# bevanda/Learning-Based-MPC

Measured on AMD Instinct MI355X. Metric: QP-steps/s (whole node) at N=20 Moore-Greitzer; KKT-residual vs MATLAB ref, higher is better.
Workload: dtype f64; 1 GPU; C2: MG LMPC (F1) N=20, 616-row terminal set, batch 1024 per GPU, fp64; batch_per_gpu=1024, horizon=20, parallelism=dp1, streams=1

## Files before the change

### learning-based-mpc_amd/csrc/bqp_api.cpp

```cpp
#include <hip/hip_runtime.h>
#include <math.h>
#include <stdio.h>
#include <stdlib.h>
#include <string.h>

#include <algorithm>
#include <vector>

#include "../../include/bqp.h"
#include "bqp_internal.h"
#include "bqp_layout.h"

namespace layout = bqp::layout;

struct DevBuf {
    void* p = nullptr;
    size_t bytes = 0;
    hipError_t reserve(size_t n) {
        if (n <= bytes) return hipSuccess;
        if (p) hipFree(p);
        p = nullptr;
        bytes = 0;
        hipError_t e = hipMalloc(&p, n);
        if (e == hipSuccess) bytes = n;
// ... 268 lines not shown
    auto shared_layout = [&](bool single) {
        Shared o;
        o.lng = !single && N + 1 > 64;
        o.hpsh = mp > 0 && D->shp == 0;
        o.bndsh = o.lng && D->sxb == 0 && D->sub == 0;
        const int nbr = (N + 1) * 2 * (nx + nu);
        int sh = (o.lng || hinst) ? 0 : (N + 1) * hstride;
        o.sh_F = sh;
        sh += fpi ? 0 : nv * mpad;
        o.sh_hp = o.hpsh ? sh : -1;
        sh += o.hpsh ? mpad : 0;
        o.sh_bnd = o.bndsh ? sh : -1;
        sh += o.bndsh ? nbr : 0;
        o.doubles = (sh + 1) & ~1;
        return o;
    };
    const Shared L64 = shared_layout(f32), L32 = shared_layout(true);
    const bool lng = L64.lng;
    auto fit_wpb = [&](bool single, int& wpb) -> bool {
        const Shared& S = single ? L32 : L64;
        const int shared_doubles = S.doubles;
        const int per_wave = single ? bqp::ocp_wave_lds_doubles_f32(N, nx, nu, np, mpad, fpi, false, S.hpsh, false, hinst)
                                    : bqp::ocp_wave_lds_doubles(N, nx, nu, np, mpad, fpi, S.lng, S.hpsh, S.bndsh, hinst);
        const size_t lds_budget = (160 * 1024 - 256) / (single ? sizeof(float) : sizeof(double));
        wpb = (N + 1 > 64) ? 2 : 4;
        if (const char* e = getenv("BQP_OCP_WPB")) {
            const int v = atoi(e);
            if (v >= 1 && v <= 8) wpb = v;
        }
        while (wpb > 1 && (size_t)shared_doubles + (size_t)wpb * per_wave > lds_budget) --wpb;
        return (size_t)shared_doubles + (size_t)per_wave <= lds_budget;
    };
    int wpb = 1, wpb32 = 1;
    if (!fit_wpb(f32, wpb)) return BQP_E_UNSUPPORTED;
    if (mixed && !fit_wpb(true, wpb32)) return BQP_E_UNSUPPORTED;
    const layout::Work WL = work_layout(N, nv, mpad, batch);
    HIP_TRY(h->work.reserve(WL.bytes));
    double* Hd = layout::at<double>(h->work.p, WL.H);
    double* Fd = layout::at<double>(h->work.p, WL.F);
    double* Sd = layout::at<double>(h->work.p, WL.stats);
    int* polneed = layout::at<int>(h->work.p, WL.marks);
    int* queues = layout::at<int>(h->work.p, WL.queues);
    const double* Hinst = nullptr;
    if (hinst) {
        HIP_TRY(h->wwork.reserve(sizeof(double) * (size_t)batch * (N + 1) * hstride));
        HIP_TRY(bqp::launch_ocp_prep_h(D->W, D->sW, batch, nx, nu, np, N, hstride, (double*)h->wwork.p, st));
        Hinst = (const double*)h->wwork.p;
    }
    void* Pg = nullptr;
    if (lng) {
        HIP_TRY(h->pwork.reserve(sizeof(double) * (size_t)batch * (N + 1) * bqp::ocp_pstride(nx + np)));
        Pg = h->pwork.p;
    }
    HIP_TRY(bqp::launch_ocp_prep(D->W, mp > 0 ? D->Fp : D->W, nx, nu, np, N, mp, d->poly_stage,
                                 hstride, mpad, Hd, Fd, queues, st));
    bqp::OcpKernelArgs a;
    memset(&a, 0, sizeof(a));
    a.queue = queues;
    a.N = N; a.mp = mp; a.kp = d->poly_stage; a.batch = batch; a.wpb = wpb;
    const Shared& LS = f32 ? L32 : L64;
    a.hstride = hstride; a.mpad = mpad; a.shared_doubles = LS.doubles;
    a.Pg = Pg; a.sh_F = LS.sh_F; a.sh_hp = LS.sh_hp; a.sh_bnd = LS.sh_bnd; a.H_inst = Hinst;
    a.max_iter = o.max_iter; a.tol_stat = o.tol_stat; a.tol_feas = o.tol_feas;
    a.tol_comp = o.tol_comp; a.tau = o.tau;
    a.polish = o.polish < 0 ? 0 : (o.polish == 0 ? 1 : std::min(o.polish, 2));
    a.pol_need = polneed;
    a.H = Hd; a.Fp = Fd;
    a.A = D->A; a.B = D->B; a.c = D->c; a.w = D->w; a.xlb = D->xlb; a.xub = D->xub;
    a.ulb = D->ulb; a.uub = D->uub; a.hp = mp > 0 ? D->hp : Hd; a.x0 = D->x0;
    a.sA = D->sA; a.sB = D->sB; a.sc = D->sc; a.sw = D->sw; a.sxb = D->sxb; a.sub = D->sub;
    a.shp = D->shp; a.sx0 = D->sx0;
    if (fpi) { a.Fp_inst = D->Fp; a.sFp = D->sFp; }
    a.x = x; a.u = u; a.theta = theta; a.fval = fval; a.exitflag = exitflag; a.stats = Sd;
    if (duals) {
        a.pi_out = duals->pi; a.lamx_out = duals->lam_x; a.lamu_out = duals->lam_u;
        a.lamp_out = duals->lam_p;
    }
#ifdef BQP_STAMPS
    a.stamps = layout::at<double>(h->work.p, WL.stamps);
    h->last_batch = batch;
#endif
    HIP_TRY(hipEventRecord(h->ev0, st));
    if (mixed) {
        const int hf = bqp::ocp_hand_floats(N, nx, nu, np, mp);
        if (hf <= 0) return BQP_E_UNSUPPORTED;
        const layout::Hwork HL(hf, batch);
        const size_t hrec = HL.stride;
        HIP_TRY(h->hwork.reserve(HL.bytes));
        float* hb = layout::at<float>(h->hwork.p, HL.records);
        int* hflag = layout::at<int>(h->hwork.p, HL.flags);
        int* hit = layout::at<int>(h->hwork.p, HL.iters);
        int* c2flag = layout::at<int>(h->hwork.p, HL.cont);
        h->mixed_flags = hflag;
        h->mixed_cont = c2flag;
        h->mixed_batch = batch;
        bqp::OcpKernelArgs a1 = a;
        a1.wpb = wpb32;
        a1.shared_doubles = L32.doubles; a1.sh_F = L32.sh_F; a1.sh_hp = L32.sh_hp; a1.sh_bnd = L32.sh_bnd;
        a1.max_iter = o32.max_iter; a1.tol_stat = o32.tol_stat; a1.tol_feas = o32.tol_feas;
        a1.tol_comp = o32.tol_comp;
        a1.exitflag = hflag;
        a1.hand_out = hb; a1.hand_it = hit; a1.hand_stride = (int64_t)hrec;
        a1.pi_out = a1.lamx_out = a1.lamu_out = a1.lamp_out = nullptr;
        a1.queue = queues + 1;
        HIP_TRY(bqp::launch_ocp_f32(a1, nx, nu, np, st));
        a.hand_in = hb; a.hand_flag = hflag; a.hand_it = hit; a.hand_stride = (int64_t)hrec;
        HIP_TRY(bqp::launch_ocp(a, nx, nu, np, st));
        HIP_TRY(hipMemcpyAsync(c2flag, exitflag, sizeof(int) * batch, hipMemcpyDeviceToDevice, st));
        bqp::OcpKernelArgs a3 = a;
        a3.hand_in = nullptr; a3.hand_it = nullptr; a3.redo_flag = hflag;
        a3.queue = nullptr;
        HIP_TRY(bqp::launch_ocp(a3, nx, nu, np, st));
    } else if (f32) {
        HIP_TRY(bqp::launch_ocp_f32(a, nx, nu, np, st));
    } else {
        HIP_TRY(bqp::launch_ocp(a, nx, nu, np, st));
    }
    if (!f32 && a.polish > 0) HIP_TRY(bqp::launch_ocp(a, nx, nu, np, st, true));
    HIP_TRY(hipEventRecord(h->ev1, st));
    h->timed = true;
// ... 675 lines not shown
```

### learning-based-mpc_amd/csrc/bqp_internal.h

```cpp
#pragma once
#include <hip/hip_runtime.h>
#include <stdint.h>

namespace bqp {

constexpr int STATS_W = 7;

constexpr int OCP_QUEUES = 4;
struct OcpKernelArgs {
    int N, mp, kp, batch, wpb, hstride, mpad, shared_doubles, max_iter;
    int* queue;
    double tol_stat, tol_feas, tol_comp, tau;
    const double* H;
    const double* Fp;
    const double *A, *B, *c, *w, *xlb, *xub, *ulb, *uub, *hp, *x0;
    int64_t sA, sB, sc, sw, sxb, sub, shp, sx0;
    double *x, *u, *theta, *fval;
    int* exitflag;
    double* stats;
    double *pi_out, *lamx_out, *lamu_out, *lamp_out;
    double* stamps;
    float* hand_out;
    const float* hand_in;
    const int* hand_flag;
    int* hand_it;
    int64_t hand_stride;
    const int* redo_flag;
    const double* Fp_inst;
    int64_t sFp;
    void* Pg;
    int sh_F, sh_hp, sh_bnd;
    const double* H_inst;
    int polish;
    int* pol_need;
};

bool ocp_supported(int nx, int nu, int np);
int ocp_rpl_for(int mp);
int ocp_bpl_for(int N, int nx, int nu);
int ocp_hand_floats(int N, int nx, int nu, int np, int mp);
int ocp_wave_lds_doubles(int N, int nx, int nu, int np, int mpad, bool fpi, bool lng, bool hpsh,
                         bool bndsh, bool hinst);
int ocp_pstride(int ns);
hipError_t launch_ocp(const OcpKernelArgs& a, int nx, int nu, int np, hipStream_t st, bool pol = false);
int ocp_wave_lds_doubles_f32(int N, int nx, int nu, int np, int mpad, bool fpi, bool lng,
                             bool hpsh, bool bndsh, bool hinst);
hipError_t launch_ocp_f32(const OcpKernelArgs& a, int nx, int nu, int np, hipStream_t st, bool pol = false);
hipError_t launch_ocp_prep(const double* W, const double* Fp, int nx, int nu, int np, int N,
                           int mp, int kp, int hstride, int mpad, double* Hout, double* Fout,
                           int* qzero, hipStream_t st);
hipError_t launch_ocp_prep_h(const double* W, int64_t sW, int batch, int nx, int nu, int np,
                             int N, int hstride, double* Hout, hipStream_t st);
hipError_t launch_ocp_finalize(const double* stats, int batch, void* out, hipStream_t st);

struct DenseKernelArgs {
    int n, m, me, batch, max_iter, mrows;
    double tol_stat, tol_feas, tol_comp, tau;
    const double *H, *f, *A, *b, *Aeq, *beq, *lb, *ub;
    int64_t sH, sf, sA, sb, sAeq, sbeq, slb, sub;
    double *x, *fval, *lam_ineqlin, *lam_eqlin, *lam_lower, *lam_upper;
    int* exitflag;
    double* stats;
    double* work;
    int64_t work_stride;
    int polish;
    const int* pol_it;
    int pol_stall;
    const int* skip;
    int res_every;
};

int dense_work_doubles(int n, int m, int me);
hipError_t launch_dense(const DenseKernelArgs& a, hipStream_t st);
hipError_t launch_dense_symmetrize(double* H, int n, int count, int64_t stride, hipStream_t st);

struct LbmpcArgs {
    int N, n, nr, m, q, n_run, term_learned, batch, ntrial, max_iter, wrows;
    double hinv2, lam_nw, tol_step, tol_stat;
    const double *A, *B, *K, *Lq, *Lr, *Lp, *Lt, *LAM, *PSI, *xs;
    const double* data; int64_t sdata;
    const double* x0; int64_t sx0;
    const double* Ain;
    const double* bin; int64_t sbin;
    double* z;
    double* d;
    double* lam;
    double *Jr, *er;
    double *H, *f, *bsh;
    double *cost0, *costT, *stat, *cprev;
    int *qpflag, *flag, *done, *iters, *ndone;
    int hess;
    double *Jr2, *Tr2;
    int* hused;
};

hipError_t launch_nw_oracle(int batch, int q, const double* data, int64_t sdata, const double* xi,
                            double* g, double* dg, double bw, double lam, hipStream_t st);
bool lbmpc_hess_fits(int n);
bool lbmpc_supported(int nx, int nu, int np, int n, int q);
hipError_t launch_lbmpc_rollout(const LbmpcArgs& a, int gn, hipStream_t st);
hipError_t launch_lbmpc_normal(const LbmpcArgs& a, hipStream_t st);
hipError_t launch_lbmpc_update(const LbmpcArgs& a, hipStream_t st);
hipError_t launch_lbmpc_hess(const LbmpcArgs& a, hipStream_t st);
// ... 29 lines not shown
```

### learning-based-mpc_amd/csrc/bqp_ocp.hip

```cpp
#include <hip/hip_runtime.h>
#include <math.h>
#include <stdint.h>
#include <stdlib.h>

#include "bqp_internal.h"
#include "bqp_lanes.h"
#include "bqp_wave.h"

namespace bqp {

#ifdef BQP_F32
typedef float real;
typedef float2 real2;
#define BQP_SFX _f32
namespace sp {
#else
typedef double real;
typedef double2 real2;
#define BQP_SFX
namespace dp {
#endif
#define BQP_CAT2(a, b) a##b
#define BQP_CAT(a, b) BQP_CAT2(a, b)

// ... 557 lines not shown
        for (int t = 0; t < VPL; ++t) {
            o.h[t] = BQP_HV(vr[t] * NV + vc[t]);
            o.d[t] = W[L.Dx + k * NV + vr[t]];
        }
    };
    auto ht = [&](int k, const HRaw& o, int t) __attribute__((always_inline)) -> real {
        real v = o.h[t] + (vr[t] == vc[t] ? o.d[t] : real(0));
        if (k == kp) v += W[L.FD + vr[t] * NV + vc[t]];
        return v;
    };
    real pu[PST];
    auto read_p = [&](int k) __attribute__((always_inline)) {
        wave_sync();
        const real2* src = reinterpret_cast<const real2*>(W + L.P + (LNG ? (k & 1) : k) * PST);
#pragma unroll
        for (int q = 0; q < PST / 2; ++q) {
            const real2 t2 = src[q];
            pu[2 * q] = t2.x;
            pu[2 * q + 1] = t2.y;
        }
    };
    auto Pm = [&](int a_, int b_) __attribute__((always_inline)) -> real { return pu[pk_idx(NS, a_, b_)]; };
    auto factor = [&]() __attribute__((always_inline)) -> bool {
        HRaw raw, nxt;
        {
            load_h(N, raw);
            const real v0 = ht(N, raw, 0);
            if (fquad && fql == 0) {
                W[L.P + (LNG ? (N & 1) : N) * PST + fq] = v0;
                if constexpr (LNG) Pgl[N * PST + fq] = v0;
            }
        }
        read_p(N);
        bool ok = true;
        auto fstage = [&](int k, const HRaw& raw) __attribute__((always_inline)) {
            real mv[VPL];
#pragma unroll
            for (int t = 0; t < VPL; ++t) {
                real sp0 = 0, sp1 = 0, sp2 = 0, sp3 = 0;
#pragma unroll
                for (int m = 0; m < NPK; ++m) {
                    if ((m & 3) == 0) sp0 = fmar(cf[t][m], pu[m], sp0);
                    if ((m & 3) == 1) sp1 = fmar(cf[t][m], pu[m], sp1);
                    if ((m & 3) == 2) sp2 = fmar(cf[t][m], pu[m], sp2);
                    if ((m & 3) == 3) sp3 = fmar(cf[t][m], pu[m], sp3);
                }
                mv[t] = ht(k, raw, t) + ((sp0 + sp1) + (sp2 + sp3));
            }
            real g[VAL];
#pragma unroll
            for (int v = 0; v < VAL; ++v) {
                const int s = v & 3;
                const real src = mv[v >> 2];
                g[v] = (s == 0) ? dpp_mov<0x00, 0xf>(real(0), src)
                     : (s == 1) ? dpp_mov<0x55, 0xf>(real(0), src)
                     : (s == 2) ? dpp_mov<0xAA, 0xf>(real(0), src)
                                : dpp_mov<0xFF, 0xf>(real(0), src);
            }
            real pv, Kc[NU], Lf[NU * NU];
            if constexpr (NU == 1) {
                ok = ok && (g[3] > 0.0);
                const real rinv = frcp(g[3]);
                Lf[0] = rinv;
                pv = fmar(-(g[1] * rinv), g[2], g[0]);
                Kc[0] = -(g[2] * rinv);
            } else {
                real Mu[NU][NU], Lc[NU][NU];
                {
                    int t = 2 * NU + 1;
#pragma unroll
                    for (int x = 0; x < NU; ++x)
#pragma unroll
                        for (int y = x; y < NU; ++y, ++t) { Mu[x][y] = g[t]; Mu[y][x] = g[t]; }
                }
                ok = chol_small<NU>(Mu, Lc) && ok;
#pragma unroll
                for (int x = 0; x < NU; ++x)
#pragma unroll
                    for (int y = 0; y < NU; ++y) Lf[x * NU + y] = Lc[x][y];
                real y[NU];
#pragma unroll
                for (int x = 0; x < NU; ++x) y[x] = g[1 + NU + x];
                chol_solve_small<NU>(Lf, y);
                real acc = g[1] * y[0];
#pragma unroll
                for (int x = 1; x < NU; ++x) acc = fmar(g[1 + x], y[x], acc);
                pv = g[0] - acc;
#pragma unroll
                for (int x = 0; x < NU; ++x) Kc[x] = -y[x];
            }
            if (fquad && fql == 0) {
                W[L.P + (LNG ? (k & 1) : k) * PST + fq] = pv;
                if constexpr (LNG) Pgl[k * PST + fq] = pv;
                if (ie == je) {
#pragma unroll
                    for (int x = 0; x < NU; ++x) W[L.K + k * NU * NS + x * NS + je] = Kc[x];
                }
                if (fq == 0) {
#pragma unroll
                    for (int x = 0; x < NU * NU; ++x) W[L.Lr + k * NU * NU + x] = Lf[x];
                }
            }
            read_p(k);
        };
        if constexpr (LNG) {
            HRaw r0, r1, r2;
            load_h(N - 1, r0);
            if (N >= 2) load_h(N - 2, r1);
            for (int k = N - 1; k >= 0; k -= 3) {
                if (k >= 2) load_h(k - 2, r2);
// ... 208 lines not shown
                    e -= W[L.ebox + (kk * NB + NX + i) * 2 + 1];
                }
                qu[j][i] = e;
            }
            if (k == kp) {
#pragma unroll
                for (int i = 0; i < NS; ++i) qs[j][i] += gpe[i];
                if (kp < N) {
#pragma unroll
                    for (int i = 0; i < NU; ++i) qu[j][i] += gpe[NS + i];
                }
            }
        }
#pragma unroll
        for (int j = 0; j < SPL; ++j) {
            const int k = stage_of(lane, j);
            if (k < N) {
                const real* Kk = W + L.K + k * NU * NS;
#pragma unroll
                for (int i = 0; i < NS; ++i) {
                    real qq = qs[j][i];
#pragma unroll
                    for (int x = 0; x < NU; ++x) MADD(qq, Kk[x * NS + i], qu[j][x]);
                    W[L.qt_xpi + k * NS + i] = qq + W[L.wv + k * NS + i];
                }
#pragma unroll
                for (int x = 0; x < NU; ++x) W[L.qu + k * NU + x] = qu[j][x];
            } else if (k == N) {
#pragma unroll
                for (int i = 0; i < NS; ++i) W[L.pv + N * NS + i] = qs[j][i];
            }
        }
        }
        wave_sync();
        STAMP(10);
        {
            real Acol[NS], Bl[NS][NU];
#pragma unroll
            for (int c = 0; c < NS; ++c) {
                Acol[c] = Abar(c, li);
#pragma unroll
                for (int x = 0; x < NU; ++x) Bl[c][x] = Bbar(c, x);
            }
            real p[NS];
#pragma unroll
            for (int i = 0; i < NS; ++i) p[i] = W[L.pv + N * NS + i];
            auto load_b = [&](int k, real (&kc)[NU], real& q) __attribute__((always_inline)) {
                q = W[L.qt_xpi + k * NS + li];
#pragma unroll
                for (int x = 0; x < NU; ++x) kc[x] = W[L.K + k * NU * NS + x * NS + li];
            };
            real k0[NU], q0, k1[NU], q1;
            load_b(N - 1, k0, q0);
            if (N >= 2) load_b(N - 2, k1, q1);
            auto step_b = [&](int k, const real (&kc)[NU], real q) __attribute__((always_inline)) {
                real acc = q;
#pragma unroll
                for (int c = 0; c < NS; ++c) {
                    real ph = Acol[c];
#pragma unroll
                    for (int x = 0; x < NU; ++x) ph += Bl[c][x] * kc[x];
                    acc += ph * p[c];
                }
                if (lane < NS) W[L.pv + k * NS + lane] = acc;
                rbc_all<0, NS>(acc, p);
            };
            for (int k = N - 1; k >= 0; k -= 2) {
                step_b(k, k0, q0);
                if (k >= 2) load_b(k - 2, k0, q0);
                if (k == 0) break;
                step_b(k - 1, k1, q1);
                if (k >= 3) load_b(k - 3, k1, q1);
            }
        }
        wave_sync();
        STAMP(11);
        if constexpr (G > 1) {
            const lanes::StageLane sl = lanes::stage_lane(lane, N, G);
            const int k = sl.k;
            if (k < N) {
                real y[NS], r[NU];
#pragma unroll
                for (int i = 0; i < NS; ++i) y[i] = W[L.pv + (k + 1) * NS + i];
#pragma unroll
                for (int x = 0; x < NU; ++x) {
                    real v = qu[0][x] + W[L.bw + k * NU + x];
#pragma unroll
                    for (int c = 0; c < NS; ++c) MADD(v, Bbar(c, x), y[c]);
                    r[x] = -v;
                }
                chol_solve_small<NU>(W + L.Lr + k * NU * NU, r);
#pragma unroll
                for (int x = 0; x < NU; ++x) kff[0][x] = r[x];
#pragma unroll
                for (int t = 0; t < ES; ++t) {
                    const int i = lanes::entry(NS, G, sl.g, t);
                    real v = W[L.re + k * NS + i];
#pragma unroll
                    for (int x = 0; x < NU; ++x) MADD(v, Bbar(i, x), kff[0][x]);
                    W[L.fv + k * NS + i] = v;
                }
            }
        } else {
#pragma unroll
        for (int j = 0; j < SPL; ++j) {
            const int k = stage_of(lane, j);
            if (k < N) {
                real y[NS], r[NU];
#pragma unroll
                for (int i = 0; i < NS; ++i) y[i] = W[L.pv + (k + 1) * NS + i];
#pragma unroll
                for (int x = 0; x < NU; ++x) {
                    real v = qu[j][x] + W[L.bw + k * NU + x];
#pragma unroll
                    for (int c = 0; c < NS; ++c) MADD(v, Bbar(c, x), y[c]);
                    r[x] = -v;
                }
                chol_solve_small<NU>(W + L.Lr + k * NU * NU, r);
#pragma unroll
                for (int x = 0; x < NU; ++x) kff[j][x] = r[x];
#pragma unroll
                for (int i = 0; i < NS; ++i) {
                    real v = LNG ? re_at(j, k, i) : W[L.re + k * NS + i];
#pragma unroll
                    for (int x = 0; x < NU; ++x) MADD(v, Bbar(i, x), kff[j][x]);
                    W[L.fv + k * NS + i] = v;
                }
            }
        }
        }
        wave_sync();
        STAMP(12);
        {
            real d[NS];
#pragma unroll
            for (int i = 0; i < NX; ++i) d[i] = 0.0;
            real r0[NP];
#pragma unroll
            for (int x = 0; x < NP; ++x) r0[x] = -W[L.pv + NX + x];
            chol_solve_small<NP>(W + L.L0, r0);
#pragma unroll
            for (int x = 0; x < NP; ++x) d[NX + x] = r0[x];
            if (lane == 0) {
#pragma unroll
                for (int i = 0; i < NS; ++i) W[ods + i] = d[i];
            }
            real Arow[NS], Bli[NU];
#pragma unroll
            for (int c = 0; c < NS; ++c) Arow[c] = Abar(li, c);
#pragma unroll
            for (int x = 0; x < NU; ++x) Bli[x] = Bbar(li, x);
            auto load_f = [&](int k, real (&kr)[NU][NS], real& f) __attribute__((always_inline)) {
                f = W[L.fv + k * NS + li];
#pragma unroll
                for (int x = 0; x < NU; ++x)
#pragma unroll
                    for (int c = 0; c < NS; ++c) kr[x][c] = W[L.K + k * NU * NS + x * NS + c];
            };
            real k0[NU][NS], f0, k1[NU][NS], f1;
            load_f(0, k0, f0);
            if (N >= 2) load_f(1, k1, f1);
            auto step_f = [&](int k, const real (&kr)[NU][NS], real f) __attribute__((always_inline)) {
                real acc = f;
#pragma unroll
                for (int c = 0; c < NS; ++c) {
                    real ph = Arow[c];
#pragma unroll
                    for (int x = 0; x < NU; ++x) ph += Bli[x] * kr[x][c];
                    acc += ph * d[c];
                }
                if (lane < NS) W[ods + (k + 1) * NS + lane] = acc;
                rbc_all<0, NS>(acc, d);
            };
            for (int k = 0; k < N; k += 2) {
                step_f(k, k0, f0);
                if (k + 2 < N) load_f(k + 2, k0, f0);
                if (k + 1 >= N) break;
                step_f(k + 1, k1, f1);
                if (k + 3 < N) load_f(k + 3, k1, f1);
            }
        }
        wave_sync();
        STAMP(13);
#pragma unroll
        for (int j = 0; j < SPL; ++j) {
            const int k = stage_of(lane, j);
            if (k < N) {
                const real* Kk = W + L.K + k * NU * NS;
#pragma unroll
                for (int x = 0; x < NU; ++x) {
                    real v = kff[j][x];
#pragma unroll
                    for (int c = 0; c < NS; ++c) MADD(v, Kk[x * NS + c], W[ods + k * NS + c]);
                    W[odu + k * NU + x] = v;
                }
            } else if (k == N) {
#pragma unroll
                for (int x = 0; x < NU; ++x) W[odu + N * NU + x] = 0.0;
            }
        }
        wave_sync();
        STAMP(14);
    };

    auto dual_dir = [&](int ids) __attribute__((always_inline)) {
        const int lane = opq(lane_w);
#pragma unroll
        for (int j = 0; j < SPL; ++j) {
            const int k = stage_of(lane, j);
            if (k > N || k < 1) continue;
            real dsk[NS];
#pragma unroll
            for (int i = 0; i < NS; ++i) dsk[i] = W[ids + k * NS + i];
            real Pk_[LNG ? PST : 1];
            const real* Pk = W + L.P + k * PST;
            if constexpr (LNG) { load_pk(k, Pk_); Pk = Pk_; }
#pragma unroll
            for (int i = 0; i < NS; ++i) {
                real v = W[L.pv + k * NS + i];
#pragma unroll
                for (int c = 0; c < NS; ++c) MADD(v, Pk[pk_idx(NS, i, c)], dsk[c]);
                W[L.wv + k * NS + i] = v;
            }
        }
    };
    auto update_stage_dir = [&](real al, int ids, int idu) __attribute__((always_inline)) {
        const int lane = opq(lane_w);
#pragma unroll
        for (int j = 0; j < SPL; ++j) {
            const int k = stage_of(lane, j);
            if (k > N) continue;
            if (k >= 1) {
#pragma unroll
// ... 800 lines not shown
                lp[q] += al * dl;
#pragma unroll
                for (int c = 0; c < NV; ++c) gpp[c] += f[c] * lp[q];
                cs += tp[q] * lp[q];
                if constexpr (BQP_POLISH) cm = fmax(cm, tp[q] * lp[q]);
                const real d = lp[q] * frcp(tp[q]);
                int idx = 0;
#pragma unroll
                for (int i2 = 0; i2 < NV; ++i2) {
                    const real di = d * f[i2];
#pragma unroll
                    for (int j2 = i2; j2 < NV; ++j2) fdt[idx++] += di * f[j2];
                }
            }
        }
        fe = wmax(fe);
        if (lane == 0) X[X_FEASB] = fe;
        constexpr int NT = NV * (NV + 1) / 2;
        real red[NV + NT + 1];
#pragma unroll
        for (int c = 0; c < NV; ++c) red[c] = gpp[c];
#pragma unroll
        for (int c = 0; c < NT; ++c) red[NV + c] = fdt[c];
        red[NV + NT] = cs;
        const real tot = wsum_t(red, lane);
        if (lane < NV) {
            W[L.gpp + lane] = tot;
        } else if (lane < NV + NT) {
            W[fd_off(0)] = tot;
            W[fd_off(1)] = tot;
        } else if (lane == NV + NT) {
            X[X_CS] = tot;
        }
        if constexpr (BQP_POLISH) {
            cm = wmax(cm);
            if (lane == 0) X[X_CMAX] = cm;
        }
    };

    auto rhs_corr_finish = [&](real smu, real tot) __attribute__((always_inline)) {
        if constexpr (LNG) {
#pragma unroll
            for (int pv = 0; pv < BPL / 2; ++pv) {
                real add = 0.0;
                if (bpres(2 * pv)) add += smu * frcp(tx[2 * pv]);
                if (bpres(2 * pv + 1)) add -= smu * frcp(tx[2 * pv + 1]);
                if (binrange(2 * pv)) W[L.ebox + lane + WAVE * pv] += add;
            }
        } else {
#pragma unroll
            for (int b = 0; b < BPL; ++b)
                if (bpres(b)) W[L.ebox + brow(b)] += smu * frcp(tx[b]);
        }
        const real other = dpp_mov<0xB1, 0xf>(real(0), tot);
        if (lane < 2 * NV && (lane & 1) == 0) W[L.gpe + lane / 2] = tot + smu * other;
    };
    auto rhs_drop_soc = [&]() __attribute__((always_inline)) {
        if constexpr (LNG) {
#pragma unroll
            for (int pv = 0; pv < BPL / 2; ++pv) {
                real add = 0.0;
                if (bpres(2 * pv)) add += box_pred_raw(2 * pv) * frcp(tx[2 * pv]);
                if (bpres(2 * pv + 1)) add -= box_pred_raw(2 * pv + 1) * frcp(tx[2 * pv + 1]);
                if (binrange(2 * pv)) W[L.ebox + lane + WAVE * pv] += add;
            }
        } else {
#pragma unroll
            for (int b = 0; b < BPL; ++b)
                if (bpres(b)) W[L.ebox + brow(b)] += box_pred_raw(b) * frcp(tx[b]);
        }
        real gc[NV];
#pragma unroll
        for (int c = 0; c < NV; ++c) gc[c] = 0.0;
#pragma unroll
        for (int q = 0; q < RPL; ++q) {
            const int r = lane + WAVE * q;
            if (r >= mp) continue;
            const real e = W[L.prp + r] * frcp(tp[q]);
#pragma unroll
            for (int c = 0; c < NV; ++c) gc[c] += Fs[c * mpad + r] * e;
        }
        const real tot = wsum_t(gc, lane);
        wave_sync();
        if (lane < NV) W[L.gpe + lane] += tot;
        wave_sync();
    };

    constexpr int HR_T = 0, HR_L = BPL * WAVE, HP_T = 2 * BPL * WAVE, HP_L = (2 * BPL + RPL) * WAVE;
    if (hand_warm<(BPL >= 16), POL>(a, inst)) {
        const float* hb = a.hand_in + (int64_t)inst * a.hand_stride + hand_rows_off(N, NS, NU);
#pragma unroll
        for (int b = 0; b < BPL; ++b) {
            tx[b] = (real)hb[HR_T + b * WAVE + lane];
            lx[b] = (real)hb[HR_L + b * WAVE + lane];
        }
#pragma unroll
        for (int q = 0; q < RPL; ++q) {
            tp[q] = (real)hb[HP_T + q * WAVE + lane];
            lp[q] = (real)hb[HP_L + q * WAVE + lane];
        }
        BARRIER();
        row_residuals();
        lam_side();
    } else {
    lam_side();
    BARRIER();
    row_residuals();
// ... 447 lines not shown
                        if (lane == 0) { X[X_ALPHA] = al; X[X_CGD] = (real)nxt; }
                        BARRIER();
                    } else {
                        BARRIER();
                        pol_tables(1);
                        BARRIER();
                        BARRIER();
                        const real va = act_res(false);
                        const int nxt = (va >= POL_STAG * va_prev) ? 2 : ((j + 1 < POL_CG && va > tol14) ? 1 : 2);
                        va_prev = va;
                        if (lane == 0) X[X_CGD] = (real)nxt;
                        BARRIER();
                    }
                }
                mode = 1;
            }
            STAMP_STORE(16);
            return;
        }
    }
    out_duals(lx, lp);

    STAMP_STORE(16);
}
#undef RP

template <int NX, int NU, int NP, int SPL, int RPL, int BPL, bool POL, bool QUEUE, int G>
__device__ __forceinline__ void ocp_body(const OcpKernelArgs& a) {
    constexpr int NS = NX + NP;
    constexpr int NV = NS + NU;
    extern __shared__ __attribute__((aligned(16))) unsigned char lds_raw[];
    real* lds = reinterpret_cast<real*>(lds_raw);
    const int N = a.N;
    const int lane_k = threadIdx.x & 63;
    const int wid = QUEUE ? __builtin_amdgcn_readfirstlane(threadIdx.x >> 6) : (threadIdx.x >> 6);
    const int qpb = a.wpb;
    if constexpr (POL) {
        const int i0 = blockIdx.x * a.wpb + ((threadIdx.x >> 6) % a.wpb);
        const bool need = i0 < a.batch && a.pol_need[i0] != 0;
        if (!__syncthreads_or(need)) return;
    }
    if constexpr (SPL == 2 && !QUEUE) {
        if (a.redo_flag) {
            const int i0 = blockIdx.x * a.wpb + ((threadIdx.x >> 6) % a.wpb);
            const bool need = i0 < a.batch && a.exitflag[i0] != 1 &&
                              (a.redo_flag[i0] == 1 || a.redo_flag[i0] == 0);
            if (!__syncthreads_or(need)) return;
        }
    }
    constexpr bool LNG = BQP_LNG_OK && SPL == 2;
    const bool fpi = a.Fp_inst != nullptr;
    real* Hs = lds;
    real* Fs = lds + a.sh_F;
    if (!LNG && !a.H_inst)
        for (int i = threadIdx.x; i < (N + 1) * a.hstride; i += blockDim.x) Hs[i] = a.H[i];
    if (!fpi)
        for (int i = threadIdx.x; i < NV * a.mpad; i += blockDim.x) Fs[i] = a.Fp[i];
    if (a.sh_hp >= 0)
        for (int r = threadIdx.x; r < a.mp; r += blockDim.x) lds[a.sh_hp + r] = a.hp[r];
    if (LNG && a.sh_bnd >= 0) {
        constexpr int NB = NX + NU;
        for (int r = threadIdx.x; r < (N + 1) * NB * 2; r += blockDim.x) {
            const int vi = r >> 1, h = r & 1, k = vi / NB, sl = vi - k * NB;
            double bd = h ? -INFINITY : INFINITY;
            if (sl < NX) {
                const double* xb = h ? a.xlb : a.xub;
                if (k > 0 && xb) bd = xb[(int64_t)k * NX + sl];
            } else {
                const double* ub_ = h ? a.ulb : a.uub;
                if (k < N && ub_) bd = ub_[(int64_t)k * NU + (sl - NX)];
            }
            lds[a.sh_bnd + r] = (real)bd;
        }
    }
    __syncthreads();
    const bool rowwave = wid >= qpb;
    const int slot0 = rowwave ? wid - qpb : wid;
    auto instance = [&](int inst, int slot, int lane, int xnext) __attribute__((always_inline)) {
        const QpLds L = QpLds::make(N, NX, NU, NP, a.mpad, fpi, LNG, a.sh_hp >= 0,
                                    LNG && a.sh_bnd >= 0, a.H_inst != nullptr);
        real* W = lds + a.shared_doubles + slot * L.total;
        real* Fsi = Fs;
        if (fpi && rowwave) {
            Fsi = W + L.Fi;
            const double* Fg = a.Fp_inst + (int64_t)inst * a.sFp;
            for (int r = lane; r < a.mpad; r += WAVE) {
#pragma unroll
                for (int c = 0; c < NV; ++c) {
                    const int e = c < NX ? c : (c < NS ? NX + NU + (c - NX) : NX + (c - NS));
                    real v = (r < a.mp) ? (real)Fg[(int64_t)e * a.mp + r] : real(0);
                    if (a.kp == N && c >= NS) v = 0;
                    Fsi[c * a.mpad + r] = v;
                }
            }
            wave_sync();
        }
        if (rowwave && lane == 0)
            *reinterpret_cast<int*>(W + L.xch + X_NEXT + xnext) = atomicAdd(a.queue, 1) + (int)gridDim.x * qpb;
#if defined(BQP_EXP_ONLY)
        if (BQP_EXP_ONLY == 1) stage_wave<NX, NU, NP, SPL, POL, G>(a, W, L, Hs, lane, inst, blockIdx.x * qpb + slot0);
        else row_wave<NX, NU, NP, BPL, RPL, POL>(a, W, L, Fsi, lds, lane, inst);
#else
        if (!rowwave)
            stage_wave<NX, NU, NP, SPL, POL, G>(a, W, L, Hs, lane, inst, blockIdx.x * qpb + slot0);
        else
            row_wave<NX, NU, NP, BPL, RPL, POL>(a, W, L, Fsi, lds, lane, inst);
#endif
        return W + L.xch;
    };
    if constexpr (!QUEUE) {
// ... 55 lines not shown
#endif
template <int NX, int NU, int NP, int SPL, int RPL, int BPL, int G>
__global__ void __launch_bounds__(SPL == 2 ? 256 : ((BQP_DI_OCC3 && NX == 2) ? 640 : 512),
                                  (BQP_DI_OCC3 && NX == 2 && SPL == 1) ? 3 : 1)
ocp_queue_kernel(OcpKernelArgs a) {
    ocp_body<NX, NU, NP, SPL, RPL, BPL, false, true, G>(a);
}

}

#if !defined(BQP_FAMILY)
#define BQP_FAM_MG 1
#define BQP_FAM_DI 1
#elif BQP_FAMILY == 1
#define BQP_FAM_MG 1
#define BQP_FAM_DI 0
#else
#define BQP_FAM_MG 0
#define BQP_FAM_DI 1
#endif

static hipError_t lds_attr(const void* k, size_t lds) {
    hipFuncAttributes fa;
    hipError_t e = hipFuncGetAttributes(&fa, k);
    if (e == hipSuccess && lds + fa.sharedSizeBytes > 160 * 1024) e = hipErrorInvalidValue;
    if (e == hipSuccess && lds > 64 * 1024)
        e = hipFuncSetAttribute(k, hipFuncAttributeMaxDynamicSharedMemorySize, (int)lds);
    if (e != hipSuccess) (void)hipGetLastError();
    return e;
}

template <int NX, int NU, int NP, int SPL, int RPL, int BPL, int G = 1>
static hipError_t launch_t(const OcpKernelArgs& a0, int blocks, size_t lds, hipStream_t st, bool pol) {
#ifdef BQP_F32
    (void)pol;
    auto k = sp::ocp_ipm_kernel<NX, NU, NP, SPL, RPL, BPL, G>;
    auto kq = sp::ocp_queue_kernel<NX, NU, NP, SPL, RPL, BPL, G>;
#else
    auto k = pol ? dp::ocp_polish_kernel<NX, NU, NP, SPL, RPL, BPL, G> : dp::ocp_ipm_kernel<NX, NU, NP, SPL, RPL, BPL, G>;
    auto kq = dp::ocp_queue_kernel<NX, NU, NP, SPL, RPL, BPL, G>;
#endif
    OcpKernelArgs a = a0;
    const bool no_queue = getenv("BQP_NO_QUEUE") != nullptr;
    if (!pol && !a.redo_flag && !a.hand_in && a.queue && !no_queue) {
        int dev = 0, cus = 0, per_cu = 0;
        hipError_t e = hipGetDevice(&dev);
        if (e == hipSuccess) e = hipDeviceGetAttribute(&cus, hipDeviceAttributeMultiprocessorCount, dev);
        if (e == hipSuccess) e = lds_attr((const void*)kq, lds);
        if (e == hipSuccess)
            e = hipOccupancyMaxActiveBlocksPerMultiprocessor(&per_cu, (const void*)kq, 128 * a.wpb, lds);
        if (e != hipSuccess) return e;
        const int resident = cus * (per_cu > 0 ? per_cu : 1);
        if (blocks > resident) {
            hipLaunchKernelGGL(kq, dim3(resident), dim3(128 * a.wpb), lds, st, a);
            return hipGetLastError();
        }
    }
    a.queue = nullptr;
    if (hipError_t e = lds_attr((const void*)k, lds)) return e;
    hipLaunchKernelGGL(k, dim3(blocks), dim3(128 * a.wpb), lds, st, a);
    return hipGetLastError();
}

template <int NX, int NU, int NP, int SPL, int BPL, int G>
static hipError_t launch_rpl_g(const OcpKernelArgs& a, int rpl, int blocks, size_t lds, hipStream_t st, bool pol) {
    switch (rpl) {
        case 1: return launch_t<NX, NU, NP, SPL, 1, BPL, G>(a, blocks, lds, st, pol);
        case 4: return launch_t<NX, NU, NP, SPL, 4, BPL, G>(a, blocks, lds, st, pol);
        case 10: return launch_t<NX, NU, NP, SPL, 10, BPL, G>(a, blocks, lds, st, pol);
        case 16: return launch_t<NX, NU, NP, SPL, 16, BPL, G>(a, blocks, lds, st, pol);
        default: return hipErrorInvalidValue;
    }
}

[[maybe_unused]] static inline int lane_groups_cap() {
    const char* e = getenv("BQP_OCP_LANE_GROUPS");
    const int v = e ? atoi(e) : lanes::MAX_GROUPS;
    return v >= 1 && v <= lanes::MAX_GROUPS ? v : lanes::MAX_GROUPS;
}

template <int NX, int NU, int NP, int SPL, int BPL>
static hipError_t launch_rpl(const OcpKernelArgs& a, int rpl, int blocks, size_t lds, hipStream_t st, bool pol) {
    constexpr int NS = NX + NP;
    constexpr int GM = (SPL == 1 && BPL == 4 && lanes::compiled(NS, NU, 3)) ? 3 : 1;
    if constexpr (GM > 1) {
        if (lanes::groups_for(a.N, NS, NU, BPL, lane_groups_cap()) == GM)
            return launch_rpl_g<NX, NU, NP, SPL, BPL, GM>(a, rpl, blocks, lds, st, pol);
    }
    return launch_rpl_g<NX, NU, NP, SPL, BPL, 1>(a, rpl, blocks, lds, st, pol);
}

template <int NX, int NU, int NP>
static hipError_t launch_spl(const OcpKernelArgs& a, int spl, int rpl, int blocks, size_t lds, hipStream_t st, bool pol) {
    const int nbr = (a.N + 1) * 2 * (NX + NU);
    if (spl == 1 && nbr <= 4 * WAVE) return launch_rpl<NX, NU, NP, 1, 4>(a, rpl, blocks, lds, st, pol);
    if (spl == 1 && nbr <= 10 * WAVE) return launch_rpl<NX, NU, NP, 1, 10>(a, rpl, blocks, lds, st, pol);
    if (spl == 2 && nbr <= 16 * WAVE) return launch_rpl<NX, NU, NP, 2, 16>(a, rpl, blocks, lds, st, pol);
    if (spl == 2 && nbr <= 20 * WAVE) return launch_rpl<NX, NU, NP, 2, 20>(a, rpl, blocks, lds, st, pol);
    return hipErrorInvalidValue;
}

hipError_t BQP_CAT(launch_ocp_mg, BQP_SFX)(const OcpKernelArgs& a, int spl, int rpl, int blocks, size_t lds, hipStream_t st, bool pol);
hipError_t BQP_CAT(launch_ocp_di, BQP_SFX)(const OcpKernelArgs& a, int spl, int rpl, int blocks, size_t lds, hipStream_t st, bool pol);

#if BQP_FAM_MG
hipError_t BQP_CAT(launch_ocp_mg, BQP_SFX)(const OcpKernelArgs& a, int spl, int rpl, int blocks, size_t lds, hipStream_t st, bool pol) {
// ... 83 lines not shown
```

### learning-based-mpc_amd/csrc/bqp_prep.hip

```cpp
#include <hip/hip_runtime.h>
#include <math.h>

#include <algorithm>

#include "../../include/bqp.h"
#include "bqp_internal.h"

namespace bqp {

__device__ __forceinline__ int ext_index(int i, int nx, int nu, int np) {
    const int ns = nx + np;
    if (i < nx) return i;
    if (i < ns) return nx + nu + (i - nx);
    return nx + (i - ns);
}

__global__ void ocp_prep_kernel(const double* __restrict__ W, const double* __restrict__ Fp,
                                int nx, int nu, int np, int N, int mp, int kp, int hstride,
                                int mpad, double* __restrict__ Hout, double* __restrict__ Fout,
                                int* __restrict__ qzero) {
    const int nv = nx + nu + np, ns = nx + np;
    if (qzero && blockIdx.x == 0 && threadIdx.x < OCP_QUEUES) qzero[threadIdx.x] = 0;
    const int nH = (N + 1) * hstride;
    const int nF = nv * mpad;
    for (int t = blockIdx.x * blockDim.x + threadIdx.x; t < nH + nF; t += gridDim.x * blockDim.x) {
        if (t < nH) {
            const int k = t / hstride, e = t % hstride;
            double v = 0.0;
            if (e < nv * nv) {
                const int i = e / nv, j = e % nv;
                const int ei = ext_index(i, nx, nu, np), ej = ext_index(j, nx, nu, np);
                v = W[(size_t)k * nv * nv + (size_t)ej * nv + ei];
                if (k == N && (i >= ns || j >= ns)) v = 0.0;
            }
            Hout[t] = v;
        } else {
            const int q = t - nH;
            const int c = q / mpad, r = q % mpad;
            double v = 0.0;
            if (r < mp) {
                v = Fp[(size_t)ext_index(c, nx, nu, np) * mp + r];
                if (kp == N && c >= ns) v = 0.0;
            }
            Fout[q] = v;
        }
    }
}

hipError_t launch_ocp_prep(const double* W, const double* Fp, int nx, int nu, int np, int N,
                           int mp, int kp, int hstride, int mpad, double* Hout, double* Fout,
                           int* qzero, hipStream_t st) {
    const int total = (N + 1) * hstride + (nx + nu + np) * mpad;
    const int blocks = (total + 255) / 256;
    hipLaunchKernelGGL(ocp_prep_kernel, dim3(blocks), dim3(256), 0, st, W, Fp, nx, nu, np, N,
                       mp, kp, hstride, mpad, Hout, Fout, qzero);
    return hipGetLastError();
}

__global__ void ocp_prep_h_kernel(const double* __restrict__ W, int64_t sW, int batch, int nx,
                                  int nu, int np, int N, int hstride, double* __restrict__ Hout) {
    const int nv = nx + nu + np, ns = nx + np;
    const int64_t per = (int64_t)(N + 1) * hstride;
    for (int64_t t = (int64_t)blockIdx.x * blockDim.x + threadIdx.x; t < per * batch;
         t += (int64_t)gridDim.x * blockDim.x) {
        const int64_t b = t / per;
        const int q = (int)(t - b * per);
        const int k = q / hstride, e = q % hstride;
        double v = 0.0;
        if (e < nv * nv) {
            const int i = e / nv, j = e % nv;
            const int ei = ext_index(i, nx, nu, np), ej = ext_index(j, nx, nu, np);
            v = W[b * sW + (int64_t)k * nv * nv + (int64_t)ej * nv + ei];
            if (k == N && (i >= ns || j >= ns)) v = 0.0;
        }
        Hout[t] = v;
    }
}

hipError_t launch_ocp_prep_h(const double* W, int64_t sW, int batch, int nx, int nu, int np,
                             int N, int hstride, double* Hout, hipStream_t st) {
    const int64_t total = (int64_t)(N + 1) * hstride * batch;
    const int blocks = (int)std::min<int64_t>((total + 255) / 256, 65536);
    hipLaunchKernelGGL(ocp_prep_h_kernel, dim3(blocks), dim3(256), 0, st, W, sW, batch, nx, nu, np,
                       N, hstride, Hout);
    return hipGetLastError();
}

__global__ void finalize_kernel(const double* __restrict__ stats, int batch, bqp_output* out) {
    const int b = blockIdx.x * blockDim.x + threadIdx.x;
    if (b >= batch) return;
    const double* s = stats + (size_t)b * STATS_W;
    bqp_output o;
    o.iterations = (int)s[0];
    o.firstorderopt = s[1];
    o.constrviolation = s[2];
    o.mu = s[3];
    o.kkt[0] = s[1];
    o.kkt[1] = s[4];
    o.kkt[2] = s[5];
    o.kkt[3] = s[3];
    o.polished = (int)s[6];
    out[b] = o;
}

hipError_t launch_ocp_finalize(const double* stats, int batch, void* out, hipStream_t st) {
    hipLaunchKernelGGL(finalize_kernel, dim3((batch + 255) / 256), dim3(256), 0, st, stats, batch,
                       (bqp_output*)out);
    return hipGetLastError();
}

}
// ... 1 lines not shown
```

### learning-based-mpc_amd/csrc/bqp_wave.h

```cpp
#pragma once
#include <hip/hip_runtime.h>
#include <math.h>

namespace bqp {

__device__ __forceinline__ void wave_sync() {
    __builtin_amdgcn_fence(__ATOMIC_RELEASE, "wavefront");
    __builtin_amdgcn_wave_barrier();
    __builtin_amdgcn_fence(__ATOMIC_ACQUIRE, "wavefront");
}

template <int CTRL, int ROWM>
__device__ __forceinline__ double dpp_mov(double old, double v) {
    const int2 o = __builtin_bit_cast(int2, old);
    const int2 x = __builtin_bit_cast(int2, v);
    int2 r;
    r.x = __builtin_amdgcn_update_dpp(o.x, x.x, CTRL, ROWM, 0xf, false);
    r.y = __builtin_amdgcn_update_dpp(o.y, x.y, CTRL, ROWM, 0xf, false);
    return __builtin_bit_cast(double, r);
}
__device__ __forceinline__ double lane63(double v) {
    const int2 x = __builtin_bit_cast(int2, v);
    int2 r;
    r.x = __builtin_amdgcn_readlane(x.x, 63);
    r.y = __builtin_amdgcn_readlane(x.y, 63);
    return __builtin_bit_cast(double, r);
}
__device__ __forceinline__ double wsum(double v) {
    v += dpp_mov<0xB1, 0xf>(0.0, v);
    v += dpp_mov<0x4E, 0xf>(0.0, v);
    v += dpp_mov<0x141, 0xf>(0.0, v);
    v += dpp_mov<0x140, 0xf>(0.0, v);
    v += dpp_mov<0x142, 0xa>(0.0, v);
    v += dpp_mov<0x143, 0xc>(0.0, v);
    return lane63(v);
}
__device__ __forceinline__ double wmax(double v) {
    v = fmax(v, dpp_mov<0xB1, 0xf>(-INFINITY, v));
    v = fmax(v, dpp_mov<0x4E, 0xf>(-INFINITY, v));
    v = fmax(v, dpp_mov<0x141, 0xf>(-INFINITY, v));
    v = fmax(v, dpp_mov<0x140, 0xf>(-INFINITY, v));
    v = fmax(v, dpp_mov<0x142, 0xa>(-INFINITY, v));
    v = fmax(v, dpp_mov<0x143, 0xc>(-INFINITY, v));
    return lane63(v);
}
__device__ __forceinline__ double wmin(double v) { return -wmax(-v); }
__device__ __forceinline__ double rl(double v, int src) {
    const int2 x = __builtin_bit_cast(int2, v);
    int2 r;
    r.x = __builtin_amdgcn_readlane(x.x, src);
    r.y = __builtin_amdgcn_readlane(x.y, src);
    return __builtin_bit_cast(double, r);
}

__device__ __forceinline__ void pl16_swap(double& a, double& b) {
    const int2 A = __builtin_bit_cast(int2, a), B = __builtin_bit_cast(int2, b);
    const auto x = __builtin_amdgcn_permlane16_swap((unsigned)A.x, (unsigned)B.x, false, false);
    const auto y = __builtin_amdgcn_permlane16_swap((unsigned)A.y, (unsigned)B.y, false, false);
    a = __builtin_bit_cast(double, make_int2((int)x[0], (int)y[0]));
    b = __builtin_bit_cast(double, make_int2((int)x[1], (int)y[1]));
}
__device__ __forceinline__ void pl32_swap(double& a, double& b) {
    const int2 A = __builtin_bit_cast(int2, a), B = __builtin_bit_cast(int2, b);
    const auto x = __builtin_amdgcn_permlane32_swap((unsigned)A.x, (unsigned)B.x, false, false);
    const auto y = __builtin_amdgcn_permlane32_swap((unsigned)A.y, (unsigned)B.y, false, false);
    a = __builtin_bit_cast(double, make_int2((int)x[0], (int)y[0]));
    b = __builtin_bit_cast(double, make_int2((int)x[1], (int)y[1]));
}
__device__ __forceinline__ void pl16_swap(float& a, float& b) {
    const auto x = __builtin_amdgcn_permlane16_swap(__builtin_bit_cast(unsigned, a),
                                                    __builtin_bit_cast(unsigned, b), false, false);
    a = __builtin_bit_cast(float, (unsigned)x[0]);
    b = __builtin_bit_cast(float, (unsigned)x[1]);
}
__device__ __forceinline__ void pl32_swap(float& a, float& b) {
    const auto x = __builtin_amdgcn_permlane32_swap(__builtin_bit_cast(unsigned, a),
                                                    __builtin_bit_cast(unsigned, b), false, false);
    a = __builtin_bit_cast(float, (unsigned)x[0]);
    b = __builtin_bit_cast(float, (unsigned)x[1]);
}
template <int CTRL, int ROWM>
__device__ __forceinline__ float dpp_mov(float old, float v) {
    return __builtin_bit_cast(float, __builtin_amdgcn_update_dpp(__builtin_bit_cast(int, old),
                                                                  __builtin_bit_cast(int, v), CTRL,
                                                                  ROWM, 0xf, false));
}
__device__ __forceinline__ float lane63(float v) {
    return __builtin_bit_cast(float, __builtin_amdgcn_readlane(__builtin_bit_cast(int, v), 63));
}
__device__ __forceinline__ float wsum(float v) {
    v += dpp_mov<0xB1, 0xf>(0.0f, v);
    v += dpp_mov<0x4E, 0xf>(0.0f, v);
    v += dpp_mov<0x141, 0xf>(0.0f, v);
    v += dpp_mov<0x140, 0xf>(0.0f, v);
    v += dpp_mov<0x142, 0xa>(0.0f, v);
    v += dpp_mov<0x143, 0xc>(0.0f, v);
    return lane63(v);
}
__device__ __forceinline__ float wmax(float v) {
    v = fmaxf(v, dpp_mov<0xB1, 0xf>(-INFINITY, v));
    v = fmaxf(v, dpp_mov<0x4E, 0xf>(-INFINITY, v));
    v = fmaxf(v, dpp_mov<0x141, 0xf>(-INFINITY, v));
    v = fmaxf(v, dpp_mov<0x140, 0xf>(-INFINITY, v));
    v = fmaxf(v, dpp_mov<0x142, 0xa>(-INFINITY, v));
    v = fmaxf(v, dpp_mov<0x143, 0xc>(-INFINITY, v));
    return lane63(v);
}
__device__ __forceinline__ float wmin(float v) { return -wmax(-v); }
__device__ __forceinline__ float rl(float v, int src) {
    return __builtin_bit_cast(float, __builtin_amdgcn_readlane(__builtin_bit_cast(int, v), src));
}

template <int C>
__device__ __forceinline__ double rbc(double v) {
    return __builtin_amdgcn_update_dpp(0.0, v, 0x150 + C, 0xf, 0xf, false);
}
template <int C>
__device__ __forceinline__ float rbc(float v) {
    return __builtin_bit_cast(float, __builtin_amdgcn_update_dpp(0, __builtin_bit_cast(int, v),
                                                                 0x150 + C, 0xf, 0xf, false));
}
template <int Q>
__device__ __forceinline__ double xrow_bcast(double v) {
    double a = v, b = v;
    pl16_swap(a, b);
    double c = (Q & 1) ? b : a, d = c;
    pl32_swap(c, d);
    return (Q >> 1) ? d : c;
}

template <int C, int NC, typename T>
__device__ __forceinline__ void rbc_all(T v, T (&p)[NC]) {
    p[C] = rbc<C>(v);
    if constexpr (C + 1 < NC) rbc_all<C + 1, NC>(v, p);
}

template <int CTRL, typename T, int KI, int KO>
__device__ __forceinline__ void tsum_step(const T (&in)[KI], T (&out)[KO], bool hi) {
#pragma unroll
    for (int p = 0; p < KO; ++p) {
        const T a = in[2 * p];
        const T b = (2 * p + 1 < KI) ? in[2 * p + 1] : T(0);
        const T keep = hi ? b : a;
        const T send = hi ? a : b;
        out[p] = keep + dpp_mov<CTRL, 0xf>(T(0), send);
    }
}
template <typename T, int K>
__device__ __forceinline__ T wsum_t(const T (&v)[K], int lane) {
    static_assert(K >= 2 && K <= 32, "wsum_t: 2..32 values");
    constexpr int K1 = (K + 1) / 2, K2 = (K1 + 1) / 2, K3 = (K2 + 1) / 2, K4 = (K3 + 1) / 2;
    T w1[K1], w2[K2], w3[K3], w4[K4];
    tsum_step<0xB1>(v, w1, (lane & 1) != 0);
    tsum_step<0x4E>(w1, w2, (lane & 2) != 0);
    tsum_step<0x124>(w2, w3, (lane & 4) != 0);
    tsum_step<0x128>(w3, w4, (lane & 8) != 0);
    T a = w4[0], b = T(0);
    if constexpr (K4 > 1) b = w4[K4 - 1];
    pl16_swap(a, b);
    T c = a + b, d = c;
    pl32_swap(c, d);
    return c + d;
}

}
```

Measured before the change: 2.510 million QP-steps/s.

## Skip OCP prep launch by permuting raw tables in-kernel; use bound_ctrl DPP moves

For horizons up to 64 without per-instance H or F, the separate prep kernel that builds padded H/F tables is skipped. The main kernel now reads the raw W and Fp matrices and does the permutation and padding itself while filling LDS. A tiny queue-zero kernel is launched only when the persistent-queue path needs it. DPP moves that only need zero fill now use bound_ctrl=true, which can drop the old-value operand and its register move. The backward and forward recursion loops are restructured to remove data-dependent branches, with a tail step for odd N. The LDS fill now does an index permutation per element, which adds some setup cost in every block.

```diff
diff --git a/learning-based-mpc_amd/csrc/bqp_api.cpp b/learning-based-mpc_amd/csrc/bqp_api.cpp
--- a/learning-based-mpc_amd/csrc/bqp_api.cpp
+++ b/learning-based-mpc_amd/csrc/bqp_api.cpp
@@ -344,10 +344,15 @@
         HIP_TRY(h->pwork.reserve(sizeof(double) * (size_t)batch * (N + 1) * bqp::ocp_pstride(nx + np)));
         Pg = h->pwork.p;
     }
-    HIP_TRY(bqp::launch_ocp_prep(D->W, mp > 0 ? D->Fp : D->W, nx, nu, np, N, mp, d->poly_stage,
-                                 hstride, mpad, Hd, Fd, queues, st));
+    const char* prep_env = getenv("BQP_OCP_PREP_LAUNCH");
+    const bool raw_tables = N + 1 <= 64 && !hinst && !fpi && !(prep_env && atoi(prep_env) == 1);
+    if (!raw_tables)
+        HIP_TRY(bqp::launch_ocp_prep(D->W, mp > 0 ? D->Fp : D->W, nx, nu, np, N, mp, d->poly_stage,
+                                     hstride, mpad, Hd, Fd, queues, st));
     bqp::OcpKernelArgs a;
     memset(&a, 0, sizeof(a));
+    a.raw_tables = raw_tables ? 1 : 0;
+    a.queue_zeroed = raw_tables ? 0 : 1;
     a.queue = queues;
     a.N = N; a.mp = mp; a.kp = d->poly_stage; a.batch = batch; a.wpb = wpb;
     const Shared& LS = f32 ? L32 : L64;
@@ -357,7 +362,8 @@
     a.tol_comp = o.tol_comp; a.tau = o.tau;
     a.polish = o.polish < 0 ? 0 : (o.polish == 0 ? 1 : std::min(o.polish, 2));
     a.pol_need = polneed;
-    a.H = Hd; a.Fp = Fd;
+    a.H = raw_tables ? D->W : Hd;
+    a.Fp = raw_tables ? (mp > 0 ? D->Fp : D->W) : Fd;
     a.A = D->A; a.B = D->B; a.c = D->c; a.w = D->w; a.xlb = D->xlb; a.xub = D->xub;
     a.ulb = D->ulb; a.uub = D->uub; a.hp = mp > 0 ? D->hp : Hd; a.x0 = D->x0;
     a.sA = D->sA; a.sB = D->sB; a.sc = D->sc; a.sw = D->sw; a.sxb = D->sxb; a.sub = D->sub;
diff --git a/learning-based-mpc_amd/csrc/bqp_internal.h b/learning-based-mpc_amd/csrc/bqp_internal.h
--- a/learning-based-mpc_amd/csrc/bqp_internal.h
+++ b/learning-based-mpc_amd/csrc/bqp_internal.h
@@ -10,6 +10,8 @@
 struct OcpKernelArgs {
     int N, mp, kp, batch, wpb, hstride, mpad, shared_doubles, max_iter;
     int* queue;
+    int queue_zeroed;
+    int raw_tables;
     double tol_stat, tol_feas, tol_comp, tau;
     const double* H;
     const double* Fp;
@@ -49,6 +51,7 @@
 hipError_t launch_ocp_prep(const double* W, const double* Fp, int nx, int nu, int np, int N,
                            int mp, int kp, int hstride, int mpad, double* Hout, double* Fout,
                            int* qzero, hipStream_t st);
+hipError_t launch_ocp_queue_zero(int* q, hipStream_t st);
 hipError_t launch_ocp_prep_h(const double* W, int64_t sW, int batch, int nx, int nu, int np,
                              int N, int hstride, double* Hout, hipStream_t st);
 hipError_t launch_ocp_finalize(const double* stats, int batch, void* out, hipStream_t st);
diff --git a/learning-based-mpc_amd/csrc/bqp_ocp.hip b/learning-based-mpc_amd/csrc/bqp_ocp.hip
--- a/learning-based-mpc_amd/csrc/bqp_ocp.hip
+++ b/learning-based-mpc_amd/csrc/bqp_ocp.hip
@@ -633,10 +633,10 @@
             for (int v = 0; v < VAL; ++v) {
                 const int s = v & 3;
                 const real src = mv[v >> 2];
-                g[v] = (s == 0) ? dpp_mov<0x00, 0xf>(real(0), src)
-                     : (s == 1) ? dpp_mov<0x55, 0xf>(real(0), src)
-                     : (s == 2) ? dpp_mov<0xAA, 0xf>(real(0), src)
-                                : dpp_mov<0xFF, 0xf>(real(0), src);
+                g[v] = (s == 0) ? dpp_mov0<0x00>(src)
+                     : (s == 1) ? dpp_mov0<0x55>(src)
+                     : (s == 2) ? dpp_mov0<0xAA>(src)
+                                : dpp_mov0<0xFF>(src);
             }
             real pv, Kc[NU], Lf[NU * NU];
             if constexpr (NU == 1) {
@@ -951,7 +951,7 @@
             };
             real k0[NU], q0, k1[NU], q1;
             load_b(N - 1, k0, q0);
-            if (N >= 2) load_b(N - 2, k1, q1);
+            load_b(max(N - 2, 0), k1, q1);
             auto step_b = [&](int k, const real (&kc)[NU], real q) __attribute__((always_inline)) {
                 real acc = q;
 #pragma unroll
@@ -964,13 +964,13 @@
                 if (lane < NS) W[L.pv + k * NS + lane] = acc;
                 rbc_all<0, NS>(acc, p);
             };
-            for (int k = N - 1; k >= 0; k -= 2) {
+            for (int k = N - 1; k >= 1; k -= 2) {
                 step_b(k, k0, q0);
-                if (k >= 2) load_b(k - 2, k0, q0);
-                if (k == 0) break;
+                load_b(max(k - 2, 0), k0, q0);
                 step_b(k - 1, k1, q1);
-                if (k >= 3) load_b(k - 3, k1, q1);
-            }
+                load_b(max(k - 3, 0), k1, q1);
+            }
+            if (N & 1) step_b(0, k0, q0);
         }
         wave_sync();
         STAMP(11);
@@ -1058,7 +1058,7 @@
             };
             real k0[NU][NS], f0, k1[NU][NS], f1;
             load_f(0, k0, f0);
-            if (N >= 2) load_f(1, k1, f1);
+            load_f(min(1, N - 1), k1, f1);
             auto step_f = [&](int k, const real (&kr)[NU][NS], real f) __attribute__((always_inline)) {
                 real acc = f;
 #pragma unroll
@@ -1071,13 +1071,13 @@
                 if (lane < NS) W[ods + (k + 1) * NS + lane] = acc;
                 rbc_all<0, NS>(acc, d);
             };
-            for (int k = 0; k < N; k += 2) {
+            for (int k = 0; k + 1 < N; k += 2) {
                 step_f(k, k0, f0);
-                if (k + 2 < N) load_f(k + 2, k0, f0);
-                if (k + 1 >= N) break;
+                load_f(min(k + 2, N - 1), k0, f0);
                 step_f(k + 1, k1, f1);
-                if (k + 3 < N) load_f(k + 3, k1, f1);
-            }
+                load_f(min(k + 3, N - 1), k1, f1);
+            }
+            if (N & 1) step_f(N - 1, k0, f0);
         }
         wave_sync();
         STAMP(13);
@@ -1984,7 +1984,7 @@
             for (int b = 0; b < BPL; ++b)
                 if (bpres(b)) W[L.ebox + brow(b)] += smu * frcp(tx[b]);
         }
-        const real other = dpp_mov<0xB1, 0xf>(real(0), tot);
+        const real other = dpp_mov0<0xB1>(tot);
         if (lane < 2 * NV && (lane & 1) == 0) W[L.gpe + lane / 2] = tot + smu * other;
     };
     auto rhs_drop_soc = [&]() __attribute__((always_inline)) {
@@ -2538,10 +2538,34 @@
     const bool fpi = a.Fp_inst != nullptr;
     real* Hs = lds;
     real* Fs = lds + a.sh_F;
+    if (!LNG && a.raw_tables) {
+        constexpr int HST = NV * NV + 1, MPAD = 64 * RPL;
+        auto ext = [](int i) { return i < NX ? i : (i < NS ? NX + NU + (i - NX) : NX + (i - NS)); };
+        for (int t = threadIdx.x; t < (N + 1) * HST; t += blockDim.x) {
+            const int k = t / HST, e = t - k * HST;
+            double v = 0.0;
+            if (e < NV * NV) {
+                const int i = e / NV, j = e - i * NV;
+                v = a.H[k * (NV * NV) + ext(j) * NV + ext(i)];
+                if (k == N && (i >= NS || j >= NS)) v = 0.0;
+            }
+            Hs[t] = v;
+        }
+        for (int q = threadIdx.x; q < NV * MPAD; q += blockDim.x) {
+            const int c = q / MPAD, r = q - c * MPAD;
+            double v = 0.0;
+            if (r < a.mp) {
+                v = a.Fp[ext(c) * a.mp + r];
+                if (a.kp == N && c >= NS) v = 0.0;
+            }
+            Fs[q] = v;
+        }
+    } else {
     if (!LNG && !a.H_inst)
         for (int i = threadIdx.x; i < (N + 1) * a.hstride; i += blockDim.x) Hs[i] = a.H[i];
     if (!fpi)
         for (int i = threadIdx.x; i < NV * a.mpad; i += blockDim.x) Fs[i] = a.Fp[i];
+    }
     if (a.sh_hp >= 0)
         for (int r = threadIdx.x; r < a.mp; r += blockDim.x) lds[a.sh_hp + r] = a.hp[r];
     if (LNG && a.sh_bnd >= 0) {
@@ -2703,6 +2727,8 @@
         if (e != hipSuccess) return e;
         const int resident = cus * (per_cu > 0 ? per_cu : 1);
         if (blocks > resident) {
+            if (!a.queue_zeroed)
+                if (hipError_t ez = launch_ocp_queue_zero(a.queue, st)) return ez;
             hipLaunchKernelGGL(kq, dim3(resident), dim3(128 * a.wpb), lds, st, a);
             return hipGetLastError();
         }
diff --git a/learning-based-mpc_amd/csrc/bqp_prep.hip b/learning-based-mpc_amd/csrc/bqp_prep.hip
--- a/learning-based-mpc_amd/csrc/bqp_prep.hip
+++ b/learning-based-mpc_amd/csrc/bqp_prep.hip
@@ -57,6 +57,13 @@
     return hipGetLastError();
 }
 
+__global__ void ocp_queue_zero_kernel(int* __restrict__ q) { *q = 0; }
+
+hipError_t launch_ocp_queue_zero(int* q, hipStream_t st) {
+    hipLaunchKernelGGL(ocp_queue_zero_kernel, dim3(1), dim3(1), 0, st, q);
+    return hipGetLastError();
+}
+
 __global__ void ocp_prep_h_kernel(const double* __restrict__ W, int64_t sW, int batch, int nx,
                                   int nu, int np, int N, int hstride, double* __restrict__ Hout) {
     const int nv = nx + nu + np, ns = nx + np;
diff --git a/learning-based-mpc_amd/csrc/bqp_wave.h b/learning-based-mpc_amd/csrc/bqp_wave.h
--- a/learning-based-mpc_amd/csrc/bqp_wave.h
+++ b/learning-based-mpc_amd/csrc/bqp_wave.h
@@ -19,6 +19,14 @@
     r.y = __builtin_amdgcn_update_dpp(o.y, x.y, CTRL, ROWM, 0xf, false);
     return __builtin_bit_cast(double, r);
 }
+template <int CTRL>
+__device__ __forceinline__ double dpp_mov0(double v) {
+    const int2 x = __builtin_bit_cast(int2, v);
+    int2 r;
+    r.x = __builtin_amdgcn_update_dpp(0, x.x, CTRL, 0xf, 0xf, true);
+    r.y = __builtin_amdgcn_update_dpp(0, x.y, CTRL, 0xf, 0xf, true);
+    return __builtin_bit_cast(double, r);
+}
 __device__ __forceinline__ double lane63(double v) {
     const int2 x = __builtin_bit_cast(int2, v);
     int2 r;
@@ -27,10 +35,10 @@
     return __builtin_bit_cast(double, r);
 }
 __device__ __forceinline__ double wsum(double v) {
-    v += dpp_mov<0xB1, 0xf>(0.0, v);
-    v += dpp_mov<0x4E, 0xf>(0.0, v);
-    v += dpp_mov<0x141, 0xf>(0.0, v);
-    v += dpp_mov<0x140, 0xf>(0.0, v);
+    v += dpp_mov0<0xB1>(v);
+    v += dpp_mov0<0x4E>(v);
+    v += dpp_mov0<0x141>(v);
+    v += dpp_mov0<0x140>(v);
     v += dpp_mov<0x142, 0xa>(0.0, v);
     v += dpp_mov<0x143, 0xc>(0.0, v);
     return lane63(v);
@@ -85,14 +93,19 @@
                                                                   __builtin_bit_cast(int, v), CTRL,
                                                                   ROWM, 0xf, false));
 }
+template <int CTRL>
+__device__ __forceinline__ float dpp_mov0(float v) {
+    return __builtin_bit_cast(float, __builtin_amdgcn_update_dpp(0, __builtin_bit_cast(int, v), CTRL,
+                                                                  0xf, 0xf, true));
+}
 __device__ __forceinline__ float lane63(float v) {
     return __builtin_bit_cast(float, __builtin_amdgcn_readlane(__builtin_bit_cast(int, v), 63));
 }
 __device__ __forceinline__ float wsum(float v) {
-    v += dpp_mov<0xB1, 0xf>(0.0f, v);
-    v += dpp_mov<0x4E, 0xf>(0.0f, v);
-    v += dpp_mov<0x141, 0xf>(0.0f, v);
-    v += dpp_mov<0x140, 0xf>(0.0f, v);
+    v += dpp_mov0<0xB1>(v);
+    v += dpp_mov0<0x4E>(v);
+    v += dpp_mov0<0x141>(v);
+    v += dpp_mov0<0x140>(v);
     v += dpp_mov<0x142, 0xa>(0.0f, v);
     v += dpp_mov<0x143, 0xc>(0.0f, v);
     return lane63(v);
@@ -113,12 +126,12 @@
 
 template <int C>
 __device__ __forceinline__ double rbc(double v) {
-    return __builtin_amdgcn_update_dpp(0.0, v, 0x150 + C, 0xf, 0xf, false);
+    return __builtin_amdgcn_update_dpp(0.0, v, 0x150 + C, 0xf, 0xf, true);
 }
 template <int C>
 __device__ __forceinline__ float rbc(float v) {
     return __builtin_bit_cast(float, __builtin_amdgcn_update_dpp(0, __builtin_bit_cast(int, v),
-                                                                 0x150 + C, 0xf, 0xf, false));
+                                                                 0x150 + C, 0xf, 0xf, true));
 }
 template <int Q>
 __device__ __forceinline__ double xrow_bcast(double v) {
@@ -143,7 +156,7 @@
         const T b = (2 * p + 1 < KI) ? in[2 * p + 1] : T(0);
         const T keep = hi ? b : a;
         const T send = hi ? a : b;
-        out[p] = keep + dpp_mov<CTRL, 0xf>(T(0), send);
+        out[p] = keep + dpp_mov0<CTRL>(send);
     }
 }
 template <typename T, int K>
```

Result: faster. 2.618 million QP-steps/s (median of 6 runs) (+4.3%).
